# NidhiMishra/SR_object_detection

Hardware: AMD Instinct MI355X
Metric: images/sec YOLOv2 608x608 fp32 (higher is better)
Workload: dtype f32

## Files before the change

include/y2_hip.h:

```cpp
#ifndef Y2_HIP_H
#define Y2_HIP_H

#include <stddef.h>
#include <stdint.h>

#ifdef __cplusplus
extern "C" {
#endif

#define Y2H_OK            0
#define Y2H_EHIP         -1
#define Y2H_EINVAL       -2
#define Y2H_ENODEV       -3

typedef void *y2h_stream;
typedef void *y2h_event;
typedef void *y2h_graph;

enum { Y2H_ACT_LINEAR = 0, Y2H_ACT_LEAKY = 1, Y2H_ACT_LOGISTIC = 2, Y2H_ACT_RELU = 3,
       Y2H_ACT_RELIE = 4, Y2H_ACT_RAMP = 5, Y2H_ACT_TANH = 6, Y2H_ACT_PLSE = 7, Y2H_ACT_ELU = 8, Y2H_ACT_LOGGY = 9,
       Y2H_ACT_STAIR = 10, Y2H_ACT_HARDTAN = 11, Y2H_ACT_LHTAN = 12 };

int         y2h_device_count(void);
int         y2h_set_device(int dev);
// ... 112 lines not shown
int y2h_wino_split_plan(const y2h_conv *d, y2h_wino_split *out);
size_t y2h_wino_split_workspace_bytes(const y2h_conv *d);
int y2h_conv_winox_forward(const y2h_conv *d, y2h_stream s);
unsigned long y2h_wino_split_launches(void);

typedef struct y2h_winos {
    int eligible;
    int take;
    int form;
    long patches;
    size_t u_bytes;
} y2h_winos;
int y2h_winos_plan(const y2h_conv *d, y2h_winos *out);
int y2h_conv_winos_forward(const y2h_conv *d, y2h_stream s);
unsigned long y2h_winos_launches(void);

int y2h_maxpool(const float *x, int ldx, float *y, int ldy, int batch, int h, int w, int c,
                int size, int stride, int pad, int out_h, int out_w, y2h_stream s);
int y2h_reorg(const float *x, int ldx, float *y, int ldy, int batch, int h, int w, int c,
              int stride, int reverse, y2h_stream s);
int y2h_connected_ref(const float *x, long x_batch_stride, int ld, int hw, int c, const float *w_ref, float *y,
                      int outputs, int batch, int batch_normalize, int activation, const float *mean,
                      const double *rinv, const float *scale, const float *bias, y2h_stream s);
int y2h_detection_boxes(const float *pred, long pred_stride, int batch, int side, int num, int classes, int sqrt_flag,
                        int w, int h, float thresh, int only_objectness, float *boxes, float *probs, y2h_stream s);
int y2h_shortcut(const float *in, int ld_in, const float *add, int ld_add, float *out, int ld_out, int batch,
                 int w1, int h1, int c1, int w2, int h2, int c2, int activation, y2h_stream s);
int y2h_crop(const float *x, int ldx, float *y, int ldy, int batch, int h, int w, int c, int out_h, int out_w,
             int noadjust, int halo, y2h_stream s);
int y2h_batchnorm(const float *x, int ldx, float *y, int ldy, long pixels, int c, const float *mean, const double *rinv,
// ... 376 lines not shown
```

sr_object_detection_amd/csrc/host/y2_arena.c:

```c
#include <math.h>
#include <stdio.h>
#include <stdlib.h>
#include <string.h>
#include "y2_internal.h"
#include "y2_wino_rule.h"
#include "y2_winos_rule.h"
#include "y2_split_rule.h"

static int owns_arena(const layer *l)
{
    return l->type == CONVOLUTIONAL || l->type == CONNECTED || l->type == LOCAL || l->type == BATCHNORM || is_recurrent(l);
}

void y2_bn_slots(size_t *off, int n, size_t *mean, size_t *scale, size_t *rinv)
{
    *mean = *off; *off = align_up(*off + n * sizeof(float), 64);
    *scale = *off; *off = align_up(*off + n * sizeof(float), 64);
    *rinv = *off; *off = align_up(*off + n * sizeof(double), 64);
}

void y2_fill_rinv(double *dst, const float *var, int n)
{
    int f;
    for (f = 0; f < n; ++f) dst[f] = 1.0 / (sqrt((double)var[f]) + (double).000001f);
// ... 185 lines not shown
static void pack_winos(void *slot, const layer *l)
{
    float *up = slot;
    int co, ci, g;
    memset(up, 0, y2_winos_u_floats(l->n) * sizeof(float));
    for (co = 0; co < l->n; ++co)
        for (ci = 0; ci < l->c; ++ci) {
            float u[16];
            y2_wino_filter(l->weights + ((size_t)co * l->c + ci) * 9, u);
            for (g = 0; g < 16; ++g) up[y2_winos_u_index(co, ci, g >> 2, g & 3)] = u[g];
        }
}

static void pack_winox(void *slot, const layer *l) { y2_split_pack_u(slot, l->weights, l->n, l->c); }

static size_t wino_slot_bytes(const layer *l) { return (size_t)16 * l->n * l->c * sizeof(float); }
static size_t winox_slot_bytes(const layer *l) { return y2_split_bytes(y2_split_rows_pad(l->n), l->c); }
static size_t winos_slot_bytes(const layer *l) { return y2_winos_u_floats(l->n) * sizeof(float); }

const y2_conv_form y2_conv_forms[Y2_FORM_COUNT] = {
    [Y2_FORM_DIRECT] = { 0, NULL, NULL, y2h_conv_workspace_bytes, NULL },
    [Y2_FORM_WINO] = { 0x57494e4f, wino_slot_bytes, pack_wino, y2h_wino_workspace_bytes, y2h_conv_wino_forward },
    [Y2_FORM_WINOX] = { 0x57494e58, winox_slot_bytes, pack_winox, y2h_wino_split_workspace_bytes, y2h_conv_winox_forward },
    [Y2_FORM_WINOS] = { 0x57494e53, winos_slot_bytes, pack_winos, NULL, y2h_conv_winos_forward },
};

static void pack_dense(unsigned char *host, const network *net, int i)
{
    const layer *l = &net->layers[i];
    const y2_ldev *d = ld_of(l);
    const y2_conv_form *form = &y2_conv_forms[d->form];
    const int K = l->size * l->size * l->c, w_half = y2_half_weights(net, i);
    int co, f, q;
    if (form->pack) form->pack(host + d->off_w_packed, l);
    else pack_filters((float *)(host + d->off_w_packed), net, i, w_half);
    if (w_half) {
        float *al = (float *)(host + d->off_alpha), *be = (float *)(host + d->off_beta);
        for (f = 0; f < l->n; ++f) {
            double a = 1.0, bb = l->biases[f];
// ... 85 lines not shown
```

sr_object_detection_amd/csrc/host/y2_internal.h:

```cpp
#ifndef Y2_INTERNAL_H
#define Y2_INTERNAL_H

#include <stddef.h>
#include <stdint.h>
#include "sr_yolo2.h"
#include "y2_hip.h"

typedef struct y2_ldev {
    struct y2_engine *eng;
    int index;
    float *out;
    int out_ld;
    float *out_alloc;
    size_t out_floats;
    int placed_in;
    int alias_of;
    unsigned copy_mask;
    size_t off_w_packed, off_w_ref, off_bias, off_mean, off_scale, off_rinv;
    int has_w_ref;
    int uses_mfma;
    int form;
    int fused_pool;
    int fused_into;
    int out_half;
// ... 12 lines not shown
    int tree_best_valid;
    float *d_region;
    float *d_flat;
    float *d_halo;
    int halo_px;
    float *d_bin;
    const char *kernel;
    struct { size_t off_w, off_bias, off_mean, off_scale, off_rinv; int n, k, bn; ACTIVATION act; int form; } rd[3];
    float *d_state;
    float *d_proj;
    float *d_hist;
    float *d_zf;
    float *d_tmp;
} y2_ldev;

enum { Y2_FORM_DIRECT = 0, Y2_FORM_WINO, Y2_FORM_WINOX, Y2_FORM_WINOS, Y2_FORM_COUNT };
typedef struct y2_conv_form {
    uint64_t sig;
    size_t (*slot_bytes)(const layer *l);
    void (*pack)(void *slot, const layer *l);
    size_t (*workspace_bytes)(const y2h_conv *c);
    int (*forward)(const y2h_conv *c, y2h_stream s);
} y2_conv_form;
extern const y2_conv_form y2_conv_forms[Y2_FORM_COUNT];

enum { Y2_REC_REF = 0, Y2_REC_SKINNY = 1, Y2_REC_MFMA = 2 };

enum { Y2_LR_CONSTANT = 0, Y2_LR_STEP, Y2_LR_EXP, Y2_LR_POLY, Y2_LR_STEPS, Y2_LR_SIG, Y2_LR_RANDOM };
typedef struct {
    int policy, step, burn_in, num_steps, adam;
    float scale, gamma, power;
// ... 130 lines not shown
int y2_ingest_u8_device(network net, const unsigned char *d_frames, int h, int w, int c, int step, int swap_rb, int letterbox);

int y2_engine_build(network *net);
void y2_free_plan(network *net);
int y2_softmax_tree_check(const network *net);
int y2_act_code(ACTIVATION a);
int y2_act_in_kernel(ACTIVATION a);
int y2_act_for_kernel(ACTIVATION a);
int y2_flat_input(const network *net);
int y2_producer_of(const network *net, int i);
int y2_is_flat(const network *net, int i);
int y2_half_weights(const network *net, int i);
void y2_input_form(const network *net, y2_in_form *f);
void y2_input_view(const network *net, int i, const float **x, int *ldx);
void y2_conv_desc(const network *net, int i, y2h_conv *c, const float *x, int ldx);
int y2_conv_form_of(const y2h_conv *c, int fused_pool, char *name, size_t name_len);

void y2_bn_slots(size_t *off, int n, size_t *mean, size_t *scale, size_t *rinv);
void y2_fill_rinv(double *dst, const float *var, int n);
void y2_arena_layout(network *net);
int y2_arena_commit(network *net);
int y2_upload_weights(network *net);

int y2_rec_hidden(const layer *l);
int y2_rec_plan(network *net, int i);
size_t y2_rec_layout(y2_ldev *d, const layer *l, size_t off);
void y2_rec_pack(unsigned char *host, const y2_ldev *d, const layer *l);
size_t y2_rec_workspace_bytes(const network *net);
int y2_rec_forward(network *net, int i, const float *x);

// ... 39 lines not shown
```

sr_object_detection_amd/csrc/host/y2_plan.c:

```c
#include <math.h>
#include <stdio.h>
#include <stdlib.h>
#include <pthread.h>
#include <string.h>
#include "y2_internal.h"

void y2_free_plan(network *net)
{
    y2_engine *e = y2_engine_of(net);
    int i;
    if (!e) return;
    for (i = 0; i < net->n; ++i) {
        y2_ldev *d = ld_of(&net->layers[i]);
        if (!d) continue;
        y2h_free(d->out_alloc); d->out_alloc = NULL; d->out = NULL;
        y2h_free(d->d_region); d->d_region = NULL;
        y2h_free(d->d_flat); d->d_flat = NULL;
        y2h_free(d->d_halo); d->d_halo = NULL; d->halo_px = 0;
        y2h_free(d->d_bin); d->d_bin = NULL;
        y2h_free(d->d_state); d->d_state = NULL;
        y2h_free(d->d_proj); d->d_proj = NULL;
        y2h_free(d->d_hist); d->d_hist = NULL;
        y2h_free(d->d_zf); d->d_zf = NULL;
        y2h_free(d->d_tmp); d->d_tmp = NULL;
// ... 818 lines not shown
    return 0;
}

int y2_conv_form_of(const y2h_conv *c, int fused_pool, char *name, size_t name_len)
{
    const char *pool = fused_pool ? "+maxpool2" : "";
    y2h_wino_split x;
    y2h_wino w;
    y2h_winos s;
    if (y2h_wino_split_plan(c, &x) == 0 && x.take) { snprintf(name, name_len, "conv_winox_f32_%dx%dx%d%s", x.bm, x.bn, x.bk, pool); return Y2_FORM_WINOX; }
    if (y2h_wino_plan(c, &w) == 0 && w.take) { snprintf(name, name_len, "conv_wino_f32_%dx%dx32%s", w.bm, w.bn, pool); return Y2_FORM_WINO; }
    if (y2h_winos_plan(c, &s) == 0 && s.take) { snprintf(name, name_len, "conv_winos_f32_c%d%s", s.form, pool); return Y2_FORM_WINOS; }
    return Y2_FORM_DIRECT;
}

static int plan_conv_forms(network *net)
{
    y2_engine *e = y2_engine_of(net);
    int i;
    if (e->strict || e->half) return 0;
    for (i = 0; i < net->n; ++i) {
        layer *l = &net->layers[i];
        y2_ldev *d = ld_of(l);
        y2h_conv c;
        const float *x; int ldx;
        if (l->type != CONVOLUTIONAL || !d->uses_mfma || l->xnor) continue;
        y2_input_view(net, i, &x, &ldx);
        conv_query(net, i, &c, x, ldx);
        d->form = y2_conv_form_of(&c, d->fused_pool, d->kname, sizeof d->kname);
        if (d->form != Y2_FORM_DIRECT) d->kernel = d->kname;
    }
    return 0;
}

static int plan_timing_events(network *net)
{
    y2_engine *e = y2_engine_of(net);
    int i;
    if (e->n_ev == net->n + 1) return 0;
    if (e->ev) { for (i = 0; i < e->n_ev; ++i) y2h_event_destroy(e->ev[i]); free(e->ev); }
    e->n_ev = net->n + 1;
    e->ev = calloc(e->n_ev, sizeof(y2h_event));
    for (i = 0; i < e->n_ev; ++i) HIP_OR_ERR(y2h_event_create(&e->ev[i]));
    return 0;
// ... 25 lines not shown
```

sr_object_detection_amd/csrc/y2_conv.hip:

```cpp
#include "y2_conv_shared.hpp"
#include "y2_split_rule.h"
#include <type_traits>

template <int BM, int BN, int BK, int KS, int WM, int WN, bool XO = false, bool SKM = false, bool WG = false>
__global__ __launch_bounds__(WM *WN * 64, 2) void conv_mfma_kernel(ConvK a)
{
    static_assert(!WG || (KS == 1 && !XO && !SKM), "the Winograd GEMM is a plain 1x1 tile walk");
    constexpr int NT = WM * WN * 64;
    constexpr int LS = BK + 4;
    constexpr int CH = BK / 4;
    constexpr int RP = NT / CH;
    constexpr int PA = (BM + RP - 1) / RP, PB = (BN + RP - 1) / RP;
    constexpr int TM = BM / WM / 32, TN = BN / WN / 32;
    static_assert(TM >= 1 && TN >= 1, "wave tile must hold at least one 32x32 MFMA tile");

    extern __shared__ __attribute__((aligned(16))) float smem[];
    constexpr int BUF = (BM + BN) * LS;
    constexpr bool ES_OWN = (WM * WN == 8);
    constexpr int ES = 36;

    const int t = threadIdx.x;
    const int lane = t & 63, wv = t >> 6;
    const int wm = wv / WN, wn = wv % WN;
    const int li = lane & 31, lh = lane >> 5;
// ... 1395 lines not shown
    y2h_wino w;
    if (y2h_wino_plan(d, &w) != Y2H_OK || !w.eligible) return Y2H_OK;
    const long blocks = 16 * (tp / Y2_SPLIT_ROWS) * (y2_split_rows_pad(d->n) / Y2_SPLIT_ROWS);
    out->gemm_cost = y2_split_gemm_cost(blocks, d->c / Y2_SPLIT_BK, vb, ub, mb);
    out->split_cost = y2_split_cost(out->gemm_cost, y2_split_transform_bytes(d->batch, d->h, d->w, d->c, d->n, d->fuse_maxpool2, tp));
    out->present_cost = w.take ? w.wino_cost : w.direct_cost;
    out->take = w.take && y2_wino_wins(out->present_cost, out->split_cost);
    return Y2H_OK;
}

extern "C" size_t y2h_wino_split_workspace_bytes(const y2h_conv *d)
{
    y2h_wino_split x;
    if (y2h_wino_split_plan(d, &x) != Y2H_OK || !x.take) return 0;
    return x.v_bytes + x.m_bytes;
}

extern "C" size_t y2h_wino_workspace_bytes(const y2h_conv *d)
{
    y2h_wino w;
    if (y2h_wino_plan(d, &w) != Y2H_OK || !w.take) return 0;
    return w.v_bytes + w.m_bytes;
}

static int first_launch(const y2h_conv *d, ConvK &a, y2h_stream s)
{
    a.nchw = d->x_nchw;
    a.w = d->w_packed;
    a.npix = d->batch * d->h * d->w;
    a.xbytes = d->x_nchw ? (unsigned)((size_t)d->batch * 3 * d->h * d->w * 4) : (unsigned)((size_t)d->batch * (d->h + 2) * (d->w + 2) * d->ldx * 4);
// ... 232 lines not shown
```

sr_object_detection_amd/csrc/y2_train_bf16.hip:

```cpp
#include "y2_train_geo.hpp"
#include "y2_split_rule.h"

typedef float f32x16 __attribute__((ext_vector_type(16)));
typedef float f32x4 __attribute__((ext_vector_type(4)));
typedef unsigned u32x4 __attribute__((ext_vector_type(4)));
typedef unsigned short u16x4 __attribute__((ext_vector_type(4)));
typedef unsigned short u16x8 __attribute__((ext_vector_type(8)));
typedef __bf16 bf16x4 __attribute__((ext_vector_type(4)));
typedef __bf16 bf16x8 __attribute__((ext_vector_type(8)));

namespace {

constexpr int KB = 32;
constexpr int KG = KB / 8;
constexpr int SLAB = TB * 16 + 32;

__device__ __forceinline__ f32x4 bf16x4_f32(u16x4 b)
{
    const u32x4 u = __builtin_convertvector(b, u32x4) << 16;
    return __builtin_bit_cast(f32x4, u);
}

__device__ __forceinline__ u16x4 bf16_rn_x4(const f32x4 v, bool fin[4])
{
    const u32x4 bits = __builtin_bit_cast(u32x4, v);
    u16x4 h = __builtin_bit_cast(u16x4, __builtin_convertvector(v, bf16x4));
#pragma unroll
    for (int k = 0; k < 4; ++k) {
        const unsigned mag = bits[k] & 0x7fffffffu;
        fin[k] = mag < 0x7f800000u;
        if (fin[k] && mag >= 0x7f7f8000u) h[k] = (unsigned short)(((bits[k] >> 16) & 0x8000u) | 0x7f7fu);
    }
    return h;
}

__device__ __forceinline__ void split3_x4(const f32x4 v, u16x4 &h, u16x4 &m, u16x4 &l)
{
    bool fin[4];
    h = bf16_rn_x4(v, fin);
    f32x4 r = v - bf16x4_f32(h);
#pragma unroll
    for (int k = 0; k < 4; ++k) if (!fin[k]) r[k] = 0.f;
    m = __builtin_bit_cast(u16x4, __builtin_convertvector(r, bf16x4));
    r = r - bf16x4_f32(m);
    l = __builtin_bit_cast(u16x4, __builtin_convertvector(r, bf16x4));
}

template <int PLANES>
__device__ __forceinline__ void put_planes(unsigned char *at, const float (&v)[8])
{
    const f32x4 lo = {v[0], v[1], v[2], v[3]}, hi = {v[4], v[5], v[6], v[7]};
    if constexpr (PLANES == 1) {
        bool fin[4];
        const u16x4 a = bf16_rn_x4(lo, fin), b = bf16_rn_x4(hi, fin);
        *(u16x8 *)at = __builtin_shufflevector(a, b, 0, 1, 2, 3, 4, 5, 6, 7);
    } else {
        u16x4 h0, m0, l0, h1, m1, l1;
        split3_x4(lo, h0, m0, l0);
        split3_x4(hi, h1, m1, l1);
        *(u16x8 *)at = __builtin_shufflevector(h0, h1, 0, 1, 2, 3, 4, 5, 6, 7);
        *(u16x8 *)(at + KG * SLAB) = __builtin_shufflevector(m0, m1, 0, 1, 2, 3, 4, 5, 6, 7);
        *(u16x8 *)(at + 2 * KG * SLAB) = __builtin_shufflevector(l0, l1, 0, 1, 2, 3, 4, 5, 6, 7);
    }
}

__device__ __forceinline__ void tap_step(Tap &t, int k, int lim, int ksize, int chans)
{
    t.ok = k < lim;
    if (++t.ch == chans) {
        t.ch = 0;
        if (++t.kx == ksize) { t.kx = 0; ++t.ky; }
    }
}

template <int MODE>
__device__ __forceinline__ const float *a_run(const float *__restrict__ src, const Geo &g, const Pix &p, const Tap &t)
{
    if (!p.ok || !t.ok) return nullptr;
    if (MODE == DX) {
// ... 71 lines not shown
                rb[e] = (r < rend && j < g.J) ? bsrc[(size_t)r * g.J + j] : 0.f;
            }
        }
    };

    f32x16 acc;
#pragma unroll
    for (int v = 0; v < 16; ++v) acc[v] = 0.f;

    unsigned char *const a_put = As + a_kg * SLAB + a_row * 16, *const b_put = Bs + b_kg * SLAB + b_row * 16;
    const unsigned char *const a_get = As + lh * SLAB + (wi * 32 + li) * 16, *const b_get = Bs + lh * SLAB + (wj * 32 + li) * 16;

    if (rbeg < rend) fetch(rbeg);
    for (int r0 = rbeg; r0 < rend; r0 += KB) {
        __syncthreads();
        put_planes<PLANES>(a_put, ra);
        put_planes<PLANES>(b_put, rb);
        __syncthreads();
        if (r0 + KB < rend) fetch(r0 + KB);
#pragma unroll
        for (int ks = 0; ks < KB / 16; ++ks) {
            bf16x8 af[PLANES], bf[PLANES];
#pragma unroll
            for (int p = 0; p < PLANES; ++p) {
                af[p] = *(const bf16x8 *)(a_get + (p * KG + 2 * ks) * SLAB);
                bf[p] = *(const bf16x8 *)(b_get + (p * KG + 2 * ks) * SLAB);
            }
            if constexpr (PLANES == 1) {
                acc = __builtin_amdgcn_mfma_f32_32x32x16_bf16(af[0], bf[0], acc, 0, 0, 0);
            } else {
                constexpr int PA[6] = {2, 0, 1, 1, 0, 0}, PB[6] = {0, 2, 1, 0, 1, 0};
#pragma unroll
// ... 62 lines not shown
```

sr_object_detection_amd/darknet.py:

```python
from __future__ import annotations

import ctypes as C
import os

import numpy as np

_HERE = os.path.dirname(os.path.abspath(__file__))
LIB_PATH = os.environ.get("Y2_LIB") or os.path.join(_HERE, "libsr_yolo2.so")


class Y2Error(RuntimeError):
    pass


class Tree(C.Structure):
    _fields_ = [("leaf", C.POINTER(C.c_int)), ("n", C.c_int), ("parent", C.POINTER(C.c_int)),
                ("group", C.POINTER(C.c_int)), ("name", C.POINTER(C.c_char_p)), ("groups", C.c_int),
                ("group_size", C.POINTER(C.c_int)), ("group_offset", C.POINTER(C.c_int))]


class Box(C.Structure):
    _fields_ = [("x", C.c_float), ("y", C.c_float), ("w", C.c_float), ("h", C.c_float)]


# ... 389 lines not shown
                                 C.c_void_p, C.c_void_p]
    L.y2h_views_to_input.argtypes = [C.c_void_p, C.c_int, C.c_void_p, C.c_int, C.c_int, C.c_int, C.c_int, C.c_void_p, C.c_void_p]
    L.y2h_accumulate_rows.argtypes = [C.c_void_p, C.c_void_p, C.c_int, C.c_void_p, C.c_int, C.c_int, C.c_void_p]
    L.y2h_lrn_fast_ok.argtypes = [C.c_int, C.c_int]
    L.y2h_lrn.argtypes = [C.c_void_p, C.c_int, C.c_void_p, C.c_int, C.c_long, C.c_int, C.c_int, C.c_float, C.c_float, C.c_float,
                          C.c_int, C.c_void_p]
    L.y2h_lrn_f16.argtypes = [C.c_void_p, C.c_int, C.c_void_p, C.c_int, C.c_long, C.c_int, C.c_int, C.c_float, C.c_float, C.c_float,
                              C.c_void_p]
    L.y2h_activate_array.argtypes = [C.c_void_p, C.c_int, C.c_long, C.c_int, C.c_int, C.c_void_p]
    L.y2h_activate_copy.argtypes = [C.c_void_p, C.c_int, C.c_void_p, C.c_int, C.c_long, C.c_int, C.c_int, C.c_void_p]
    L.y2h_activate_copy_f16.argtypes = [C.c_void_p, C.c_int, C.c_void_p, C.c_int, C.c_long, C.c_int, C.c_int, C.c_void_p]
    if hasattr(L, "y2h_wino_split_plan"):
        L.y2h_wino_split_plan.argtypes = [C.c_void_p, C.c_void_p]
        L.y2h_wino_split_workspace_bytes.restype = C.c_size_t
        L.y2h_wino_split_launches.restype = C.c_ulong
    L.y2h_d2h_copies.restype = C.c_ulong
    L.y2h_stream_syncs.restype = C.c_ulong
    L.y2_set_view_block_bytes.argtypes = [C.c_size_t]
    L.y2_view_resizes.restype = C.c_ulong
    L.y2_classifier_view_sums.argtypes = [C.POINTER(CNetwork), C.c_int, C.POINTER(Image), C.c_int, C.c_void_p, C.c_int, C.c_void_p]
    L.y2_validate_classifier_10_frames.argtypes = [CNetwork, C.POINTER(Image), C.c_int, C.c_void_p, C.c_int, C.c_int,
                                                   C.POINTER(C.c_float), C.POINTER(C.c_float)]
    L.y2_validate_classifier_multi_frames.argtypes = [C.POINTER(CNetwork), C.POINTER(Image), C.c_int, C.c_void_p, C.c_int,
                                                      C.c_void_p, C.c_int, C.c_int, C.POINTER(C.c_float), C.POINTER(C.c_float)]
    L.y2_validate_classifier_full_frames.argtypes = [C.POINTER(CNetwork), C.POINTER(Image), C.c_int, C.c_void_p, C.c_int, C.c_int,
                                                     C.POINTER(C.c_float), C.POINTER(C.c_float)]
    L.y2_classify_frames.argtypes = [CNetwork, C.c_void_p, C.c_int, C.c_int, C.c_void_p, C.c_void_p]
    L.y2_hierarchy_enqueue.argtypes = [CNetwork, C.c_int]
    L.read_tree.restype = C.POINTER(Tree)
    L.read_tree.argtypes = [C.c_char_p]
# ... 1744 lines not shown
```

Baseline: 3019.

## Add split-bf16 direct 3x3 conv kernel with fused BN/leaky and optional maxpool

```diff
diff --git a/include/y2_hip.h b/include/y2_hip.h
--- a/include/y2_hip.h
+++ b/include/y2_hip.h
@@ -150,6 +150,19 @@
 int y2h_winos_plan(const y2h_conv *d, y2h_winos *out);
 int y2h_conv_winos_forward(const y2h_conv *d, y2h_stream s);
 unsigned long y2h_winos_launches(void);
+
+typedef struct y2h_splitd {
+    int eligible;
+    int take;
+    int bm, bn, bk;
+    long tiles;
+    size_t u_bytes;
+    size_t lds_bytes;
+    double direct_cost, matrix_cost, byte_cost, splitd_cost;
+} y2h_splitd;
+int y2h_conv_splitd_plan(const y2h_conv *d, y2h_splitd *out);
+int y2h_conv_splitd_forward(const y2h_conv *d, y2h_stream s);
+unsigned long y2h_conv_splitd_launches(void);
 
 int y2h_maxpool(const float *x, int ldx, float *y, int ldy, int batch, int h, int w, int c,
                 int size, int stride, int pad, int out_h, int out_w, y2h_stream s);
diff --git a/include/y2_splitd_rule.h b/include/y2_splitd_rule.h
--- /dev/null
+++ b/include/y2_splitd_rule.h
@@ -0,0 +1,88 @@
+#ifndef Y2_SPLITD_RULE_H
+#define Y2_SPLITD_RULE_H
+
+#include <stddef.h>
+#include <stdint.h>
+#include <stdio.h>
+#include <stdlib.h>
+#include <string.h>
+
+#include "y2_split_rule.h"
+
+#define Y2_SPLITD_BM 256
+#define Y2_SPLITD_UNIT_W 32
+#define Y2_SPLITD_UNIT_PITCH 34
+#define Y2_SPLITD_UNIT_POS (4 * Y2_SPLITD_UNIT_PITCH)
+#define Y2_SPLITD_LDS_BYTES 163840
+#define Y2_SPLITD_STEP_CYCLES 1536.0
+#define Y2_SPLITD_EFF 0.47
+
+static inline int y2_splitd_bn(int n, int pool)
+{
+    const char *f = getenv("Y2_SPLITD_TILE");
+    int bm = 0, bn = 0;
+    if (pool) return 128;
+    if (f && sscanf(f, "%dx%d", &bm, &bn) == 2 && bm == Y2_SPLITD_BM && (bn == 128 || bn == 256)) return bn;
+    return n <= 128 ? 128 : 256;
+}
+
+static inline int y2_splitd_shape_ok(int size, int stride, int pad, int c, int n, int h, int w, int out_h, int out_w, int pool,
+                                     int x_f16, int y_f16, int x_halo, int x_nchw, int ldx)
+{
+    if (x_f16 || y_f16 || x_halo || x_nchw) return 0;
+    if (size != 3 || stride != 1 || pad != 1 || out_h != h || out_w != w) return 0;
+    if (c <= 0 || c % Y2_SPLIT_BK != 0 || n <= 0 || n % 4 != 0 || ldx % 4 != 0) return 0;
+    if (pool && ((h | w) & 1)) return 0;
+    return 1;
+}
+
+static inline long y2_splitd_positions(int batch, int h, int w, int pool)
+{
+    if (pool) return (long)batch * (h / 2) * ((w + Y2_SPLITD_UNIT_W - 1) / Y2_SPLITD_UNIT_W) * (2 * Y2_SPLITD_UNIT_W);
+    return (long)batch * (h + 1) * (w + 2);
+}
+static inline int y2_splitd_patch_positions(int w, int pool) { return pool ? 4 * Y2_SPLITD_UNIT_POS : Y2_SPLITD_BM + 2 * (w + 3); }
+static inline long y2_splitd_tiles_m(int batch, int h, int w, int pool)
+{
+    return (y2_splitd_positions(batch, h, w, pool) + Y2_SPLITD_BM - 1) / Y2_SPLITD_BM;
+}
+
+static inline size_t y2_splitd_lds_bytes(int w, int pool, int bn)
+{
+    return (size_t)2 * y2_splitd_patch_positions(w, pool) * 96 + (size_t)3 * 96 * bn + (size_t)bn * 20;
+}
+
+static inline size_t y2_splitd_u_elems(int n, int c, int bn) { return (size_t)((n + bn - 1) / bn) * (size_t)(c / Y2_SPLIT_BK) * 9 * 48 * (size_t)bn; }
+static inline size_t y2_splitd_u_index(int c, int bn, int co, int ci, int tap, int p)
+{
+    const size_t run = ((size_t)(co / bn) * (size_t)(c / Y2_SPLIT_BK) + (size_t)(ci / Y2_SPLIT_BK)) * 9 + (size_t)tap;
+    return run * 48 * (size_t)bn + ((size_t)(p * 2 + (ci % Y2_SPLIT_BK) / 8) * (size_t)bn + (size_t)(co % bn)) * 8 + (size_t)(ci % 8);
+}
+
+static inline void y2_splitd_pack_u(uint16_t *up, const float *weights, int n, int c, int bn)
+{
+    int co, ci, tap;
+    memset(up, 0, y2_splitd_u_elems(n, c, bn) * 2);
+    for (co = 0; co < n; ++co)
+        for (ci = 0; ci < c; ++ci)
+            for (tap = 0; tap < 9; ++tap) {
+                uint16_t h, m, l;
+                y2_split3(weights[((size_t)co * c + ci) * 9 + tap], &h, &m, &l);
+                up[y2_splitd_u_index(c, bn, co, ci, tap, 0)] = h;
+                up[y2_splitd_u_index(c, bn, co, ci, tap, 1)] = m;
+                up[y2_splitd_u_index(c, bn, co, ci, tap, 2)] = l;
+            }
+}
+
+static inline double y2_splitd_matrix_cost(long tiles, int nk, int bn)
+{
+    return (double)((tiles + 255) / 256) * nk * 9.0 * Y2_SPLITD_STEP_CYCLES * (bn / 128) / Y2_SPLITD_EFF;
+}
+static inline double y2_splitd_byte_cost(double x_bytes, double halo, double u_bytes, double y_bytes)
+{
+    return (x_bytes * halo + u_bytes + y_bytes) * Y2_WINO_BYTE_CYCLES;
+}
+
+static inline double y2_splitd_halo(int w, int pool) { return (double)y2_splitd_patch_positions(w, pool) / Y2_SPLITD_BM; }
+
+#endif
diff --git a/sr_object_detection_amd/csrc/host/y2_arena.c b/sr_object_detection_amd/csrc/host/y2_arena.c
--- a/sr_object_detection_amd/csrc/host/y2_arena.c
+++ b/sr_object_detection_amd/csrc/host/y2_arena.c
@@ -5,6 +5,7 @@
 #include "y2_internal.h"
 #include "y2_wino_rule.h"
 #include "y2_winos_rule.h"
+#include "y2_splitd_rule.h"
 #include "y2_split_rule.h"
 
 static int owns_arena(const layer *l)
@@ -223,15 +224,19 @@
 
 static void pack_winox(void *slot, const layer *l) { y2_split_pack_u(slot, l->weights, l->n, l->c); }
 
+static void pack_splitd(void *slot, const layer *l) { y2_splitd_pack_u(slot, l->weights, l->n, l->c, y2_splitd_bn(l->n, ld_of(l)->fused_pool)); }
+
 static size_t wino_slot_bytes(const layer *l) { return (size_t)16 * l->n * l->c * sizeof(float); }
 static size_t winox_slot_bytes(const layer *l) { return y2_split_bytes(y2_split_rows_pad(l->n), l->c); }
 static size_t winos_slot_bytes(const layer *l) { return y2_winos_u_floats(l->n) * sizeof(float); }
+static size_t splitd_slot_bytes(const layer *l) { return y2_splitd_u_elems(l->n, l->c, y2_splitd_bn(l->n, ld_of(l)->fused_pool)) * 2; }
 
 const y2_conv_form y2_conv_forms[Y2_FORM_COUNT] = {
     [Y2_FORM_DIRECT] = { 0, NULL, NULL, y2h_conv_workspace_bytes, NULL },
     [Y2_FORM_WINO] = { 0x57494e4f, wino_slot_bytes, pack_wino, y2h_wino_workspace_bytes, y2h_conv_wino_forward },
     [Y2_FORM_WINOX] = { 0x57494e58, winox_slot_bytes, pack_winox, y2h_wino_split_workspace_bytes, y2h_conv_winox_forward },
     [Y2_FORM_WINOS] = { 0x57494e53, winos_slot_bytes, pack_winos, NULL, y2h_conv_winos_forward },
+    [Y2_FORM_SPLITD] = { 0x53504c44, splitd_slot_bytes, pack_splitd, NULL, y2h_conv_splitd_forward },
 };
 
 static void pack_dense(unsigned char *host, const network *net, int i)
diff --git a/sr_object_detection_amd/csrc/host/y2_internal.h b/sr_object_detection_amd/csrc/host/y2_internal.h
--- a/sr_object_detection_amd/csrc/host/y2_internal.h
+++ b/sr_object_detection_amd/csrc/host/y2_internal.h
@@ -50,7 +50,7 @@
     float *d_tmp;
 } y2_ldev;
 
-enum { Y2_FORM_DIRECT = 0, Y2_FORM_WINO, Y2_FORM_WINOX, Y2_FORM_WINOS, Y2_FORM_COUNT };
+enum { Y2_FORM_DIRECT = 0, Y2_FORM_WINO, Y2_FORM_WINOX, Y2_FORM_WINOS, Y2_FORM_SPLITD, Y2_FORM_COUNT };
 typedef struct y2_conv_form {
     uint64_t sig;
     size_t (*slot_bytes)(const layer *l);
@@ -211,6 +211,7 @@
 void y2_input_form(const network *net, y2_in_form *f);
 void y2_input_view(const network *net, int i, const float **x, int *ldx);
 void y2_conv_desc(const network *net, int i, y2h_conv *c, const float *x, int ldx);
+int y2_conv_layer_form(const y2h_conv *c, int fused_pool, char *name, size_t name_len);
 int y2_conv_form_of(const y2h_conv *c, int fused_pool, char *name, size_t name_len);
 
 void y2_bn_slots(size_t *off, int n, size_t *mean, size_t *scale, size_t *rinv);
diff --git a/sr_object_detection_amd/csrc/host/y2_plan.c b/sr_object_detection_amd/csrc/host/y2_plan.c
--- a/sr_object_detection_amd/csrc/host/y2_plan.c
+++ b/sr_object_detection_amd/csrc/host/y2_plan.c
@@ -856,6 +856,18 @@
     return Y2_FORM_DIRECT;
 }
 
+int y2_conv_layer_form(const y2h_conv *c, int fused_pool, char *name, size_t name_len)
+{
+    const int form = y2_conv_form_of(c, fused_pool, name, name_len);
+    y2h_splitd sd;
+    if (form != Y2_FORM_DIRECT) return form;
+    if (y2h_conv_splitd_plan(c, &sd) == 0 && sd.take) {
+        snprintf(name, name_len, "conv_splitd_f32_%dx%dx%d%s", sd.bm, sd.bn, sd.bk, fused_pool ? "+maxpool2" : "");
+        return Y2_FORM_SPLITD;
+    }
+    return Y2_FORM_DIRECT;
+}
+
 static int plan_conv_forms(network *net)
 {
     y2_engine *e = y2_engine_of(net);
@@ -869,7 +881,7 @@
         if (l->type != CONVOLUTIONAL || !d->uses_mfma || l->xnor) continue;
         y2_input_view(net, i, &x, &ldx);
         conv_query(net, i, &c, x, ldx);
-        d->form = y2_conv_form_of(&c, d->fused_pool, d->kname, sizeof d->kname);
+        d->form = y2_conv_layer_form(&c, d->fused_pool, d->kname, sizeof d->kname);
         if (d->form != Y2_FORM_DIRECT) d->kernel = d->kname;
     }
     return 0;
diff --git a/sr_object_detection_amd/csrc/y2_conv.hip b/sr_object_detection_amd/csrc/y2_conv.hip
--- a/sr_object_detection_amd/csrc/y2_conv.hip
+++ b/sr_object_detection_amd/csrc/y2_conv.hip
@@ -1,5 +1,6 @@
 #include "y2_conv_shared.hpp"
 #include "y2_split_rule.h"
+#include "y2_splitd_rule.h"
 #include <type_traits>
 
 template <int BM, int BN, int BK, int KS, int WM, int WN, bool XO = false, bool SKM = false, bool WG = false>
@@ -1433,6 +1434,44 @@
     y2h_wino_split x;
     if (y2h_wino_split_plan(d, &x) != Y2H_OK || !x.take) return 0;
     return x.v_bytes + x.m_bytes;
+}
+
+extern "C" int y2h_conv_splitd_plan(const y2h_conv *d, y2h_splitd *out)
+{
+    if (!d || !out) return Y2H_EINVAL;
+    memset(out, 0, sizeof *out);
+    int mode = -1;
+    if (const char *f = getenv("Y2_SPLITD")) mode = atoi(f) != 0 ? 1 : 0;
+    const int pool = d->fuse_maxpool2 ? 1 : 0;
+    if (!y2_splitd_shape_ok(d->size, d->stride, d->pad, d->c, d->n, d->h, d->w, d->out_h, d->out_w, pool, d->x_f16, d->y_f16,
+                            d->x_halo, d->x_nchw, d->ldx)) return Y2H_OK;
+    if (d->ldy < d->n || d->tile_bm || d->ksplit > 1 || getenv("Y2_CONV_TILE")) return Y2H_OK;
+    if (((uintptr_t)d->x | (uintptr_t)d->w_packed) % 16 != 0 || !d->w_packed) return Y2H_OK;
+    const ConvPlan p = conv_plan(d, 0);
+    if (p.kind != CK_MFMA_F32) return Y2H_OK;
+    const int bn = y2_splitd_bn(d->n, pool);
+    const double xbytes = (double)d->batch * d->h * d->w * d->ldx * 4.0;
+    const double ybytes = (double)d->batch * d->h * d->w * (pool ? 0.25 : 1.0) * d->ldy * 4.0;
+    const double ubytes = (double)y2_splitd_u_elems(d->n, d->c, bn) * 2.0;
+    if (xbytes >= 4294967000.0 || ybytes >= 4294967000.0 || ubytes >= 4294967000.0) return Y2H_OK;
+    if ((double)d->batch * (d->h + 1) * (d->w + 2) >= 1073741824.0) return Y2H_OK;
+    const size_t lds = y2_splitd_lds_bytes(d->w, pool, bn);
+    if (lds > Y2_SPLITD_LDS_BYTES || 2 * y2_splitd_patch_positions(d->w, pool) > (bn == 256 ? 2 : 3) * 512) return Y2H_OK;
+    const long tiles_n = (d->n + bn - 1) / bn, tiles = y2_splitd_tiles_m(d->batch, d->h, d->w, pool) * tiles_n;
+    if (tiles >= 0x7fffffffL / 256) return Y2H_OK;
+    out->eligible = 1;
+    out->bm = Y2_SPLITD_BM; out->bn = bn; out->bk = Y2_SPLIT_BK;
+    out->tiles = tiles;
+    out->u_bytes = (size_t)ubytes;
+    out->lds_bytes = lds;
+    out->direct_cost = p.cost;
+    out->matrix_cost = y2_splitd_matrix_cost(tiles, d->c / Y2_SPLIT_BK, bn);
+    out->byte_cost = y2_splitd_byte_cost((double)d->batch * d->h * d->w * d->c * 4.0, y2_splitd_halo(d->w, pool), ubytes,
+                                         (double)d->batch * d->h * d->w * (pool ? 0.25 : 1.0) * d->n * 4.0);
+    out->splitd_cost = out->matrix_cost > out->byte_cost ? out->matrix_cost : out->byte_cost;
+    if (mode >= 0) out->take = mode;
+    else out->take = tiles_n == 1 && bn == 128 && tiles >= 256 && p.sk_wgs == 0 && p.tile_ksplit == 1 && y2_wino_wins(p.cost, out->splitd_cost);
+    return Y2H_OK;
 }
 
 extern "C" size_t y2h_wino_workspace_bytes(const y2h_conv *d)
diff --git a/sr_object_detection_amd/csrc/y2_conv_split.hip b/sr_object_detection_amd/csrc/y2_conv_split.hip
--- /dev/null
+++ b/sr_object_detection_amd/csrc/y2_conv_split.hip
@@ -0,0 +1,317 @@
+#include "y2_conv_shared.hpp"
+#include "y2_splitd_rule.h"
+#include "y2_split_dev.hpp"
+#include <string.h>
+
+typedef __attribute__((address_space(3))) void lds_void_d;
+typedef __bf16 bf16x8 __attribute__((ext_vector_type(8)));
+
+namespace {
+
+struct SplitDK {
+    const float *x;
+    const unsigned short *u;
+    float *y;
+    const float *mean, *scale, *bias;
+    const double *rinv;
+    unsigned xbytes, ubytes, ybytes;
+    int H, W, Wp, batch, ldx, ldy, N, nk;
+    int np;
+    int pp;
+    int ux;
+    int tiles_n, ntiles;
+    int bn, act, vec_store;
+};
+
+constexpr unsigned SD_NONE = 0xffffffffu;
+
+template <int BN, bool POOL, bool FAST>
+__global__ __launch_bounds__(512, 1) void conv_splitd_kernel(SplitDK a)
+{
+    static_assert(BN == 128 || (BN == 256 && !POOL), "the pooled form has one filter tile of 128");
+    constexpr int NJ = BN / 128;
+    constexpr int RUN_B = 96 * BN;
+    constexpr int FPL_B = 32 * BN, FHALF_B = 16 * BN;
+    constexpr int PIECES = BN == 256 ? 3 : 2;
+    constexpr int NPASS = BN == 256 ? 2 : 3;
+    extern __shared__ __attribute__((aligned(16))) unsigned char sd_smem[];
+
+    const int t = threadIdx.x, lane = t & 63, l31 = lane & 31, lh = lane >> 5;
+    const int wv = __builtin_amdgcn_readfirstlane(t >> 6);
+    const int wm = wv >> 2, wn = wv & 3;
+    const bool BN_ = FAST ? true : (bool)a.bn;
+    const int ACT_ = FAST ? (int)Y2H_ACT_LEAKY : a.act;
+    const int HALF_B = a.pp * 16, PLANE_B = 2 * HALF_B, PATCH_B = 3 * PLANE_B;
+    const int pitch = POOL ? Y2_SPLITD_UNIT_PITCH : a.Wp;
+    unsigned char *fbuf = sd_smem + 2 * PATCH_B;
+    float *c_mean = (float *)(fbuf + 3 * RUN_B), *c_scale = c_mean + BN, *c_bias = c_scale + BN;
+    double *c_rinv = (double *)(c_bias + BN);
+
+    const __amdgpu_buffer_rsrc_t xr = __builtin_amdgcn_make_buffer_rsrc((void *)a.x, 0, a.xbytes, 0x00020000);
+    const __amdgpu_buffer_rsrc_t ur = __builtin_amdgcn_make_buffer_rsrc((void *)a.u, 0, a.ubytes, 0x00020000);
+    const __amdgpu_buffer_rsrc_t yr = __builtin_amdgcn_make_buffer_rsrc((void *)a.y, 0, a.ybytes, 0x00020000);
+
+    auto load_consts = [&](int tn) {
+        if (t < BN) {
+            const int f = tn * BN + t;
+            float mean = 0.f, scale = 1.f, bias = 0.f;
+            double rinv = 1.0;
+            if (f < a.N) {
+                bias = a.bias[f];
+                if (BN_) { mean = a.mean[f]; rinv = a.rinv[f]; scale = a.scale[f]; }
+            }
+            c_mean[t] = mean; c_scale[t] = scale; c_bias[t] = bias; c_rinv[t] = rinv;
+        }
+    };
+
+    unsigned s_off[NPASS];
+    auto patch_addr = [&](int tm) {
+#pragma unroll
+        for (int p = 0; p < NPASS; ++p) {
+            const int item = t + 512 * p, q = item >> 1;
+            bool ok = tm >= 0 && q < a.pp;
+            int n, y, x;
+            if (POOL) {
+                const int u = q / Y2_SPLITD_UNIT_POS, rem = q - u * Y2_SPLITD_UNIT_POS;
+                const int r = rem / Y2_SPLITD_UNIT_PITCH, ci = rem - r * Y2_SPLITD_UNIT_PITCH;
+                const int U = (tm < 0 ? 0 : tm) * 4 + u;
+                ok = ok && U < a.np;
+                const int pr = U / a.ux, xs = U - pr * a.ux;
+                const int Hp = a.H >> 1;
+                n = pr / Hp;
+                y = 2 * (pr - n * Hp) - 1 + r;
+                x = 32 * xs - 1 + ci;
+                ok = ok && y >= 0 && y < a.H && x >= 0 && x < a.W;
+            } else {
+                const int P = (tm < 0 ? 0 : tm) * Y2_SPLITD_BM - a.Wp - 1 + q;
+                ok = ok && P >= 0 && P < a.np;
+                const int Pc = P < 0 ? 0 : P;
+                const int r = Pc / a.Wp;
+                x = Pc - r * a.Wp;
+                n = r / (a.H + 1);
+                y = r - n * (a.H + 1);
+                ok = ok && x < a.W && y < a.H;
+            }
+            s_off[p] = ok ? (unsigned)((n * a.H + y) * a.W + x) * (unsigned)(a.ldx * 4) + (unsigned)(item & 1) * 32u : SD_NONE;
+        }
+    };
+    auto patch_load = [&](int p, unsigned kadd, u32x4 &r0, u32x4 &r1) {
+        const unsigned o = s_off[p] == SD_NONE ? a.xbytes : s_off[p] + kadd;
+        r0 = __builtin_amdgcn_raw_buffer_load_b128(xr, o, 0, 0);
+        r1 = __builtin_amdgcn_raw_buffer_load_b128(xr, o + 16u, 0, 0);
+    };
+    auto patch_store = [&](int p, unsigned char *buf, const u32x4 r0, const u32x4 r1) {
+        const int item = t + 512 * p, q = item >> 1;
+        if (q >= a.pp) return;
+        u16x4 h0, m0, l0, h1, m1, l1;
+        split3_x4(__builtin_bit_cast(f32x4, r0), h0, m0, l0);
+        split3_x4(__builtin_bit_cast(f32x4, r1), h1, m1, l1);
+        unsigned char *at = buf + (item & 1) * HALF_B + q * 16;
+        *(u16x8 *)at = __builtin_shufflevector(h0, h1, 0, 1, 2, 3, 4, 5, 6, 7);
+        *(u16x8 *)(at + PLANE_B) = __builtin_shufflevector(m0, m1, 0, 1, 2, 3, 4, 5, 6, 7);
+        *(u16x8 *)(at + 2 * PLANE_B) = __builtin_shufflevector(l0, l1, 0, 1, 2, 3, 4, 5, 6, 7);
+    };
+
+    auto filter_dma = [&](unsigned off, int b) {
+        unsigned char *dst = fbuf + b * RUN_B;
+        if (BN == 256) {
+#pragma unroll
+            for (int p = 0; p < 3; ++p)
+                __builtin_amdgcn_raw_ptr_buffer_load_lds(ur, (lds_void_d *)(dst + p * 8192 + wv * 1024), 16, off + p * 8192u + (unsigned)t * 16u, 0, 0, 0);
+        } else {
+            __builtin_amdgcn_raw_ptr_buffer_load_lds(ur, (lds_void_d *)(dst + wv * 1024), 16, off + (unsigned)t * 16u, 0, 0, 0);
+            __builtin_amdgcn_raw_ptr_buffer_load_lds(ur, (lds_void_d *)(dst + 8192 + (wv & 3) * 1024), 16,
+                                                     off + 8192u + (unsigned)((wv & 3) * 1024 + lane * 16), 0, 0, 0);
+        }
+    };
+
+    const unsigned u_base = (unsigned)lh * FHALF_B + (unsigned)(wn * (BN / 4) + l31) * 16u;
+    const unsigned v_base = (unsigned)lh * (unsigned)HALF_B + (unsigned)((POOL ? wm * 2 * Y2_SPLITD_UNIT_POS : wm * 128) + l31) * 16u;
+    auto v_row = [](int i) { return POOL ? (i >> 1) * Y2_SPLITD_UNIT_POS + (i & 1) * Y2_SPLITD_UNIT_PITCH : i * 32; };
+
+    const unsigned KT_B = 9u * RUN_B;
+    long tile = blockIdx.x;
+    int tm = (int)(tile / a.tiles_n), tn = (int)(tile - (long)tm * a.tiles_n);
+    unsigned f_cur = (unsigned)(tn * a.nk) * KT_B;
+
+    load_consts(tn);
+    patch_addr(tm);
+#pragma unroll
+    for (int p = 0; p < NPASS; ++p) {
+        u32x4 r0, r1;
+        patch_load(p, 0u, r0, r1);
+        patch_store(p, sd_smem, r0, r1);
+    }
+    __builtin_amdgcn_sched_barrier(0);
+    filter_dma(f_cur, 0);
+    filter_dma(f_cur + RUN_B, 1);
+    __builtin_amdgcn_sched_barrier(0);
+
+    int pb = 0;
+    for (;;) {
+        const long ntile = tile + gridDim.x;
+        const bool nlive = ntile < a.ntiles;
+        const int ntm = nlive ? (int)(ntile / a.tiles_n) : -1, ntn = nlive ? (int)(ntile - (long)ntm * a.tiles_n) : 0;
+        f32x16 acc[4][NJ];
+#pragma unroll
+        for (int i = 0; i < 4; ++i)
+#pragma unroll
+            for (int j = 0; j < NJ; ++j)
+#pragma unroll
+                for (int r = 0; r < 16; ++r) acc[i][j][r] = 0.f;
+        for (int kt = 0; kt < a.nk; ++kt) {
+            const bool last = kt + 1 == a.nk;
+            if (last) patch_addr(ntm);
+            const unsigned kadd = last ? 0u : (unsigned)(kt + 1) * 64u;
+            const unsigned f_next = last ? (unsigned)(ntn * a.nk) * KT_B : f_cur + KT_B;
+            unsigned char *nbuf = sd_smem + (pb ^ 1) * PATCH_B;
+#pragma unroll
+            for (int tap = 0; tap < 9; ++tap) {
+                if (PIECES == 3) asm volatile("s_waitcnt vmcnt(3) lgkmcnt(0)" ::: "memory");
+                else asm volatile("s_waitcnt vmcnt(2) lgkmcnt(0)" ::: "memory");
+                __builtin_amdgcn_s_barrier();
+                __builtin_amdgcn_sched_barrier(0);
+                u32x4 r0, r1;
+                if (tap < NPASS) patch_load(tap, kadd, r0, r1);
+                filter_dma(tap + 2 < 9 ? f_cur + (unsigned)(tap + 2) * RUN_B : f_next + (unsigned)(tap - 7) * RUN_B, (tap + 2) % 3);
+                __builtin_amdgcn_sched_barrier(0);
+                const unsigned char *fb = fbuf + (tap % 3) * RUN_B;
+                unsigned pa = v_base + (unsigned)(pb * PATCH_B);
+                asm volatile("" : "+v"(pa));
+                const unsigned char *pl = sd_smem + pa + (unsigned)((tap / 3) * pitch + tap % 3) * 16u;
+                bf16x8 pf[4][3], uf[NJ][3];
+                auto read_u = [&](int p) {
+#pragma unroll
+                    for (int j = 0; j < NJ; ++j) uf[j][p] = *(const bf16x8 *)(fb + u_base + p * FPL_B + j * 512);
+                };
+                auto read_p = [&](int p) {
+#pragma unroll
+                    for (int i = 0; i < 4; ++i) pf[i][p] = *(const bf16x8 *)(pl + p * PLANE_B + v_row(i) * 16);
+                };
+                auto product = [&](int pv, int pu) {
+#pragma unroll
+                    for (int i = 0; i < 4; ++i)
+#pragma unroll
+                        for (int j = 0; j < NJ; ++j)
+                            acc[i][j] = __builtin_amdgcn_mfma_f32_32x32x16_bf16(uf[j][pu], pf[i][pv], acc[i][j], 0, 0, 0);
+                };
+                read_u(0); read_p(2); read_p(0); read_u(2);
+                product(2, 0);
+                __builtin_amdgcn_sched_barrier(0);
+                read_p(1); read_u(1);
+                product(0, 2);
+                product(1, 1);
+                product(1, 0);
+                product(0, 1);
+                product(0, 0);
+                if (tap < NPASS) patch_store(tap, nbuf, r0, r1);
+            }
+            f_cur = f_next;
+            pb ^= 1;
+        }
+
+        int pix[4];
+        if (POOL) {
+            const int Hp = a.H >> 1, Wq = a.W >> 1;
+#pragma unroll
+            for (int ul = 0; ul < 2; ++ul) {
+                const int U = tm * 4 + 2 * wm + ul;
+                const int pr = U / a.ux, xs = U - pr * a.ux;
+                const int x = 32 * xs + l31;
+                pix[ul] = (U < a.np && x < a.W && !(l31 & 1)) ? pr * Wq + (x >> 1) : -1;
+                (void)Hp;
+            }
+            pix[2] = pix[3] = -1;
+        } else {
+#pragma unroll
+            for (int i = 0; i < 4; ++i) {
+                const int P = tm * Y2_SPLITD_BM + wm * 128 + i * 32 + l31;
+                const int r = P / a.Wp, x = P - r * a.Wp;
+                const int n = r / (a.H + 1), y = r - n * (a.H + 1);
+                pix[i] = (P < a.np && x < a.W && y < a.H) ? (n * a.H + y) * a.W + x : -1;
+            }
+        }
+        int fl0 = wn * (BN / 4) + lh * 4;
+        asm volatile("" : "+v"(fl0));
+#pragma unroll
+        for (int j = 0; j < NJ; ++j)
+#pragma unroll
+            for (int rg = 0; rg < 4; ++rg) {
+                const int fl = fl0 + j * 32 + rg * 8, f = tn * BN + fl;
+                const bool fok = f < a.N;
+                const f32x4 mean = *(const f32x4 *)(c_mean + fl), scale = *(const f32x4 *)(c_scale + fl), bias = *(const f32x4 *)(c_bias + fl);
+                double rinv[4];
+#pragma unroll
+                for (int e = 0; e < 4; ++e) rinv[e] = c_rinv[fl + e];
+#pragma unroll
+                for (int i = 0; i < (POOL ? 2 : 4); ++i) {
+                    f32x4 o;
+#pragma unroll
+                    for (int e = 0; e < 4; ++e) {
+                        float v;
+                        if (POOL) {
+                            const float e0 = acc[2 * i][j][4 * rg + e], o0 = acc[2 * i + 1][j][4 * rg + e];
+                            v = pool_pick(e0, __shfl_xor(e0, 1), o0, __shfl_xor(o0, 1), !BN_ || scale[e] >= 0.f);
+                        } else v = acc[i][j][4 * rg + e];
+                        o[e] = epilogue(v, BN_, mean[e], rinv[e], scale[e], bias[e], ACT_);
+                    }
+                    const bool ok = pix[i] >= 0 && fok;
+                    const unsigned idx = (unsigned)pix[i] * (unsigned)a.ldy + (unsigned)f;
+                    if (a.vec_store) __builtin_amdgcn_raw_buffer_store_b128(__builtin_bit_cast(u32x4, o), yr, ok ? idx * 4u : SD_NONE, 0, 0);
+                    else if (ok) {
+#pragma unroll
+                        for (int e = 0; e < 4; ++e) a.y[(size_t)idx + e] = o[e];
+                    }
+                    if (!FAST) __builtin_amdgcn_sched_barrier(0);
+                }
+            }
+        if (!nlive) break;
+        if (a.tiles_n > 1) {
+            asm volatile("s_waitcnt lgkmcnt(0)" ::: "memory");
+            __builtin_amdgcn_s_barrier();
+            load_consts(ntn);
+        }
+        tile = ntile; tm = ntm; tn = ntn;
+    }
+    asm volatile("s_waitcnt vmcnt(0)" ::: "memory");
+}
+
+}
+
+static unsigned long g_splitd_launches = 0;
+extern "C" unsigned long y2h_conv_splitd_launches(void) { return g_splitd_launches; }
+
+extern "C" int y2h_conv_splitd_forward(const y2h_conv *d, y2h_stream s)
+{
+    if (!conv_args_ok(d) || !d->w_packed) return Y2H_EINVAL;
+    y2h_splitd w;
+    if (y2h_conv_splitd_plan(d, &w) != Y2H_OK || !w.take) return Y2H_EINVAL;
+    const int pool = d->fuse_maxpool2 ? 1 : 0;
+    SplitDK a;
+    memset(&a, 0, sizeof a);
+    a.x = d->x; a.u = (const unsigned short *)d->w_packed; a.y = d->y;
+    a.mean = d->mean; a.rinv = d->rinv; a.scale = d->scale; a.bias = d->bias;
+    a.H = d->h; a.W = d->w; a.Wp = d->w + 2; a.batch = d->batch; a.ldx = d->ldx; a.ldy = d->ldy; a.N = d->n; a.nk = d->c / Y2_SPLIT_BK;
+    a.bn = d->batch_normalize; a.act = d->activation;
+    a.ux = (d->w + Y2_SPLITD_UNIT_W - 1) / Y2_SPLITD_UNIT_W;
+    a.np = pool ? d->batch * (d->h / 2) * a.ux : (int)y2_splitd_positions(d->batch, d->h, d->w, 0);
+    a.pp = y2_splitd_patch_positions(d->w, pool);
+    a.tiles_n = (d->n + w.bn - 1) / w.bn;
+    a.ntiles = (int)w.tiles;
+    a.xbytes = (unsigned)((size_t)d->batch * d->h * d->w * d->ldx * 4);
+    a.ubytes = (unsigned)w.u_bytes;
+    a.ybytes = (unsigned)((size_t)d->batch * d->h * d->w / (pool ? 4 : 1) * d->ldy * 4);
+    a.vec_store = d->ldy % 4 == 0 && (uintptr_t)d->y % 16 == 0;
+    const bool fast = d->batch_normalize && d->activation == Y2H_ACT_LEAKY;
+    void (*fn)(SplitDK);
+    if (w.bn == 256) fn = fast ? conv_splitd_kernel<256, false, true> : conv_splitd_kernel<256, false, false>;
+    else if (pool) fn = fast ? conv_splitd_kernel<128, true, true> : conv_splitd_kernel<128, true, false>;
+    else fn = fast ? conv_splitd_kernel<128, false, true> : conv_splitd_kernel<128, false, false>;
+    Y2H_CHECK(y2h_lds_limit((const void *)fn, w.lds_bytes));
+    long grid = w.tiles < 256 ? w.tiles : 256;
+    if (const char *g = getenv("Y2_CONV_GRID")) { if (atol(g) > 0 && atol(g) < grid) grid = atol(g); }
+    hipLaunchKernelGGL(fn, dim3((unsigned)grid), dim3(512), w.lds_bytes, S(s), a);
+    Y2H_LAUNCH_CHECK();
+    ++g_splitd_launches;
+    return Y2H_OK;
+}
diff --git a/sr_object_detection_amd/csrc/y2_split_dev.hpp b/sr_object_detection_amd/csrc/y2_split_dev.hpp
--- /dev/null
+++ b/sr_object_detection_amd/csrc/y2_split_dev.hpp
@@ -0,0 +1,61 @@
+#pragma once
+#include "y2_common.hpp"
+
+typedef float f32x4 __attribute__((ext_vector_type(4)));
+typedef unsigned u32x4 __attribute__((ext_vector_type(4)));
+typedef unsigned short u16x4 __attribute__((ext_vector_type(4)));
+typedef unsigned short u16x8 __attribute__((ext_vector_type(8)));
+typedef __bf16 bf16x4 __attribute__((ext_vector_type(4)));
+
+namespace {
+
+__device__ __forceinline__ f32x4 bf16x4_f32(u16x4 b)
+{
+    const u32x4 u = __builtin_convertvector(b, u32x4) << 16;
+    return __builtin_bit_cast(f32x4, u);
+}
+
+__device__ __forceinline__ u16x4 bf16_rn_x4(const f32x4 v, bool fin[4])
+{
+    const u32x4 bits = __builtin_bit_cast(u32x4, v);
+    u16x4 h = __builtin_bit_cast(u16x4, __builtin_convertvector(v, bf16x4));
+#pragma unroll
+    for (int k = 0; k < 4; ++k) {
+        const unsigned mag = bits[k] & 0x7fffffffu;
+        fin[k] = mag < 0x7f800000u;
+        if (fin[k] && mag >= 0x7f7f8000u) h[k] = (unsigned short)(((bits[k] >> 16) & 0x8000u) | 0x7f7fu);
+    }
+    return h;
+}
+
+__device__ __forceinline__ void split3_x4(const f32x4 v, u16x4 &h, u16x4 &m, u16x4 &l)
+{
+    bool fin[4];
+    h = bf16_rn_x4(v, fin);
+    f32x4 r = v - bf16x4_f32(h);
+#pragma unroll
+    for (int k = 0; k < 4; ++k) if (!fin[k]) r[k] = 0.f;
+    m = __builtin_bit_cast(u16x4, __builtin_convertvector(r, bf16x4));
+    r = r - bf16x4_f32(m);
+    l = __builtin_bit_cast(u16x4, __builtin_convertvector(r, bf16x4));
+}
+
+template <int PLANES, int PLANE_B>
+__device__ __forceinline__ void put_planes(unsigned char *at, const float (&v)[8])
+{
+    const f32x4 lo = {v[0], v[1], v[2], v[3]}, hi = {v[4], v[5], v[6], v[7]};
+    if constexpr (PLANES == 1) {
+        bool fin[4];
+        const u16x4 a = bf16_rn_x4(lo, fin), b = bf16_rn_x4(hi, fin);
+        *(u16x8 *)at = __builtin_shufflevector(a, b, 0, 1, 2, 3, 4, 5, 6, 7);
+    } else {
+        u16x4 h0, m0, l0, h1, m1, l1;
+        split3_x4(lo, h0, m0, l0);
+        split3_x4(hi, h1, m1, l1);
+        *(u16x8 *)at = __builtin_shufflevector(h0, h1, 0, 1, 2, 3, 4, 5, 6, 7);
+        *(u16x8 *)(at + PLANE_B) = __builtin_shufflevector(m0, m1, 0, 1, 2, 3, 4, 5, 6, 7);
+        *(u16x8 *)(at + 2 * PLANE_B) = __builtin_shufflevector(l0, l1, 0, 1, 2, 3, 4, 5, 6, 7);
+    }
+}
+
+}
diff --git a/sr_object_detection_amd/csrc/y2_train_bf16.hip b/sr_object_detection_amd/csrc/y2_train_bf16.hip
--- a/sr_object_detection_amd/csrc/y2_train_bf16.hip
+++ b/sr_object_detection_amd/csrc/y2_train_bf16.hip
@@ -1,5 +1,6 @@
 #include "y2_train_geo.hpp"
 #include "y2_split_rule.h"
+#include "y2_split_dev.hpp"
 
 typedef float f32x16 __attribute__((ext_vector_type(16)));
 typedef float f32x4 __attribute__((ext_vector_type(4)));
@@ -14,55 +15,6 @@
 constexpr int KB = 32;
 constexpr int KG = KB / 8;
 constexpr int SLAB = TB * 16 + 32;
-
-__device__ __forceinline__ f32x4 bf16x4_f32(u16x4 b)
-{
-    const u32x4 u = __builtin_convertvector(b, u32x4) << 16;
-    return __builtin_bit_cast(f32x4, u);
-}
-
-__device__ __forceinline__ u16x4 bf16_rn_x4(const f32x4 v, bool fin[4])
-{
-    const u32x4 bits = __builtin_bit_cast(u32x4, v);
-    u16x4 h = __builtin_bit_cast(u16x4, __builtin_convertvector(v, bf16x4));
-#pragma unroll
-    for (int k = 0; k < 4; ++k) {
-        const unsigned mag = bits[k] & 0x7fffffffu;
-        fin[k] = mag < 0x7f800000u;
-        if (fin[k] && mag >= 0x7f7f8000u) h[k] = (unsigned short)(((bits[k] >> 16) & 0x8000u) | 0x7f7fu);
-    }
-    return h;
-}
-
-__device__ __forceinline__ void split3_x4(const f32x4 v, u16x4 &h, u16x4 &m, u16x4 &l)
-{
-    bool fin[4];
-    h = bf16_rn_x4(v, fin);
-    f32x4 r = v - bf16x4_f32(h);
-#pragma unroll
-    for (int k = 0; k < 4; ++k) if (!fin[k]) r[k] = 0.f;
-    m = __builtin_bit_cast(u16x4, __builtin_convertvector(r, bf16x4));
-    r = r - bf16x4_f32(m);
-    l = __builtin_bit_cast(u16x4, __builtin_convertvector(r, bf16x4));
-}
-
-template <int PLANES>
-__device__ __forceinline__ void put_planes(unsigned char *at, const float (&v)[8])
-{
-    const f32x4 lo = {v[0], v[1], v[2], v[3]}, hi = {v[4], v[5], v[6], v[7]};
-    if constexpr (PLANES == 1) {
-        bool fin[4];
-        const u16x4 a = bf16_rn_x4(lo, fin), b = bf16_rn_x4(hi, fin);
-        *(u16x8 *)at = __builtin_shufflevector(a, b, 0, 1, 2, 3, 4, 5, 6, 7);
-    } else {
-        u16x4 h0, m0, l0, h1, m1, l1;
-        split3_x4(lo, h0, m0, l0);
-        split3_x4(hi, h1, m1, l1);
-        *(u16x8 *)at = __builtin_shufflevector(h0, h1, 0, 1, 2, 3, 4, 5, 6, 7);
-        *(u16x8 *)(at + KG * SLAB) = __builtin_shufflevector(m0, m1, 0, 1, 2, 3, 4, 5, 6, 7);
-        *(u16x8 *)(at + 2 * KG * SLAB) = __builtin_shufflevector(l0, l1, 0, 1, 2, 3, 4, 5, 6, 7);
-    }
-}
 
 __device__ __forceinline__ void tap_step(Tap &t, int k, int lim, int ksize, int chans)
 {
@@ -164,8 +116,8 @@
     if (rbeg < rend) fetch(rbeg);
     for (int r0 = rbeg; r0 < rend; r0 += KB) {
         __syncthreads();
-        put_planes<PLANES>(a_put, ra);
-        put_planes<PLANES>(b_put, rb);
+        put_planes<PLANES, KG * SLAB>(a_put, ra);
+        put_planes<PLANES, KG * SLAB>(b_put, rb);
         __syncthreads();
         if (r0 + KB < rend) fetch(r0 + KB);
 #pragma unroll
diff --git a/sr_object_detection_amd/darknet.py b/sr_object_detection_amd/darknet.py
--- a/sr_object_detection_amd/darknet.py
+++ b/sr_object_detection_amd/darknet.py
@@ -427,6 +427,9 @@
         L.y2h_wino_split_plan.argtypes = [C.c_void_p, C.c_void_p]
         L.y2h_wino_split_workspace_bytes.restype = C.c_size_t
         L.y2h_wino_split_launches.restype = C.c_ulong
+    if hasattr(L, "y2h_conv_splitd_plan"):
+        L.y2h_conv_splitd_plan.argtypes = [C.c_void_p, C.c_void_p]
+        L.y2h_conv_splitd_launches.restype = C.c_ulong
     L.y2h_d2h_copies.restype = C.c_ulong
     L.y2h_stream_syncs.restype = C.c_ulong
     L.y2_set_view_block_bytes.argtypes = [C.c_size_t]
```

Result: faster. 3232, median of 6 (+7.1%).
